# mll-lab-nu/TStar

Hardware: AMD Instinct MI355X
Metric: candidate frames scored/sec (whole node) + sec/video to 8 keyframes, 1h@1fps (higher is better)
Workload: dtype f32 held exactly as 3 bf16 terms per operand: every GEMM and vision-attention operand (activations, weights, Q, K, V, softmax probabilities) = three round-to-nearest bf16 terms carrying all 24 significand bits; the 6 partial products with i + j <= 2 (each exact) on v_mfma_f32_32x32x16_bf16, f32 accu

## Files before the change

### tstar_amd/csrc/attention_x3.h

```cpp
#pragma once
#include <hip/hip_runtime.h>
#include <math.h>
#include <utility>

namespace tstar {
namespace ax3 {

typedef __bf16 bf16x8 __attribute__((ext_vector_type(8)));
typedef __bf16 bf16x2 __attribute__((ext_vector_type(2)));
typedef float f32x2 __attribute__((ext_vector_type(2)));
typedef float f32x4 __attribute__((ext_vector_type(4)));
typedef float f32x16 __attribute__((ext_vector_type(16)));
typedef unsigned int u32x4 __attribute__((ext_vector_type(4)));
typedef unsigned int u32x2 __attribute__((ext_vector_type(2)));

constexpr int HD = 64, KB = 32;
constexpr int VPITCH = 80;
constexpr int KP = KB * 128, VP = HD * VPITCH;
constexpr int KBUF = 3 * KP, VBUF = 3 * VP, NKB = 2, NVB = 3;
constexpr int LDS_BYTES = NKB * KBUF + NVB * VBUF;

#define AX3_FENCE() __builtin_amdgcn_sched_barrier(0)

__device__ __forceinline__ void split2_rn3(float x0, float x1, unsigned (&o)[3]) {
#pragma unroll
    for (int k = 0; k < 3; ++k) {
        f32x2 x; x[0] = x0; x[1] = x1;
        const unsigned hb = __builtin_bit_cast(unsigned, __builtin_convertvector(x, bf16x2));
        o[k] = hb;
        if (k < 2) {
            x0 = x0 - __uint_as_float(hb << 16);
            x1 = x1 - __uint_as_float(hb & 0xFFFF0000u);
        }
    }
}
__device__ __forceinline__ float xhalf_max(float x) {
    const auto r = __builtin_amdgcn_permlane32_swap(__float_as_uint(x), __float_as_uint(x), false, false);
    return fmaxf(__uint_as_float(r[0]), __uint_as_float(r[1]));
}
__device__ __forceinline__ float xhalf_sum(float x) {
    const auto r = __builtin_amdgcn_permlane32_swap(__float_as_uint(x), __float_as_uint(x), false, false);
    return __uint_as_float(r[0]) + __uint_as_float(r[1]);
}

__device__ __forceinline__ int k_off(int key, int chunk) { return key * 128 + ((chunk ^ ((key >> 1) & 7)) << 4); }
__device__ __forceinline__ int v_off(int d, int chunk) { return d * VPITCH + (chunk << 4); }
__device__ __forceinline__ int v_keypos(int k) { const int g = k >> 2; const int gp = (g & 4) | ((g & 1) << 1) | ((g >> 1) & 1); return (gp * 4 + (k & 3)) * 2; }

__device__ __forceinline__ f32x16 mfma(const bf16x8 a, const u32x4 b, const f32x16 c) {
    return __builtin_amdgcn_mfma_f32_32x32x16_bf16(a, __builtin_bit_cast(bf16x8, b), c, 0, 0, 0);
}

template <bool PLANES>
__global__ __launch_bounds__(256, 2) void attention_x3_kernel(const float* __restrict__ qkv, const char* __restrict__ planes,
                                                              float* __restrict__ out, int T, int heads, int qtiles) {
    extern __shared__ __attribute__((aligned(16))) char smem[];
    char* const kbuf = smem;
    char* const vbuf = smem + NKB * KBUF;

    const int D = heads * HD, D3 = 3 * D;
    int bid = blockIdx.x;
    const int qt = bid % qtiles; bid /= qtiles;
    const int head = bid % heads;
    const int b = bid / heads;

    const int t = threadIdx.x, lane = t & 63, wave = __builtin_amdgcn_readfirstlane(t >> 6);
    const int l31 = lane & 31, h = lane >> 5;
    const size_t rowbase = (size_t)b * T;

    const int q = qt * 128 + wave * 32 + l31;
    const int qc = q < T ? q : T - 1;
    const bool wave_active = (qt * 128 + wave * 32) < T;

    u32x4 qp[3][4];
    {
        const float* src = qkv + (rowbase + qc) * D3 + head * HD + 8 * h;
        const float sc = 0.125f * 1.44269504088896340736f;
#pragma unroll
        for (int s = 0; s < 4; ++s) {
            const f32x4 a = *reinterpret_cast<const f32x4*>(src + 16 * s) * sc;
            const f32x4 c = *reinterpret_cast<const f32x4*>(src + 16 * s + 4) * sc;
            unsigned o0[3], o1[3], o2[3], o3[3];
            split2_rn3(a[0], a[1], o0); split2_rn3(a[2], a[3], o1); split2_rn3(c[0], c[1], o2); split2_rn3(c[2], c[3], o3);
#pragma unroll
            for (int k = 0; k < 3; ++k) { qp[k][s][0] = o0[k]; qp[k][s][1] = o1[k]; qp[k][s][2] = o2[k]; qp[k][s][3] = o3[k]; }
        }
    }

    const int kc4 = t & 15, kr = t >> 4;
    const int vkp = t & 15, vdq = t >> 4;
    const __amdgpu_buffer_rsrc_t kv_rsrc =
        __builtin_amdgcn_make_buffer_rsrc(const_cast<float*>(qkv + rowbase * D3), 0, (int)((size_t)T * D3 * 4), 0x00020000);
    int kvo[2], vvo[2];
#pragma unroll
    for (int i = 0; i < 2; ++i) {
        kvo[i] = ((kr + 16 * i) * D3 + D + head * HD + kc4 * 4) * 4;
        vvo[i] = ((2 * vkp + i) * D3 + 2 * D + head * HD + vdq * 4) * 4;
    }
    const int kwr0 = k_off(kr, kc4 >> 1) + (kc4 & 1) * 8, kwr1 = k_off(kr + 16, kc4 >> 1) + (kc4 & 1) * 8;
    int vwr[4];
#pragma unroll
    for (int e = 0; e < 4; ++e) {
        const int pos = v_keypos(2 * vkp);
        vwr[e] = v_off(4 * vdq + e, pos >> 4) + (pos & 15);
    }

    const int R0 = b * T;
    const int kt0 = R0 >> 5;
    const bool tail_key = !PLANES && (T % KB) == 1;
    const int nkb = PLANES ? ((R0 + T - 1) >> 5) - kt0 + 1 : (tail_key ? T / KB : (T + KB - 1) / KB);

    f32x4 rk[2], rv[2];
    auto gload = [&](int kb) __attribute__((always_inline)) {
        const int so = (kb < nkb ? kb : nkb) * (KB * 4) * D3;
#pragma unroll
        for (int i = 0; i < 2; ++i) {
            rk[i] = __builtin_bit_cast(f32x4, __builtin_amdgcn_raw_buffer_load_b128(kv_rsrc, kvo[i], so, 0));
            rv[i] = __builtin_bit_cast(f32x4, __builtin_amdgcn_raw_buffer_load_b128(kv_rsrc, vvo[i], so, 0));
        }
    };
    unsigned ksp[2][3];
    auto stage_piece = [&](auto P, char* kdst, char* vdst) __attribute__((always_inline)) {
        constexpr int p = decltype(P)::value;
        if constexpr (p < 4) {
            constexpr int i = p >> 1, hf = p & 1;
            split2_rn3(rk[i][2 * hf], rk[i][2 * hf + 1], ksp[hf]);
            if constexpr (hf == 1) {
#pragma unroll
                for (int k = 0; k < 3; ++k) {
                    u32x2 v; v[0] = ksp[0][k]; v[1] = ksp[1][k];
                    *reinterpret_cast<u32x2*>(kdst + k * KP + (i == 0 ? kwr0 : kwr1)) = v;
                }
            }
        } else {
            constexpr int e = p - 4;
            unsigned o[3];
            split2_rn3(rv[0][e], rv[1][e], o);
#pragma unroll
            for (int k = 0; k < 3; ++k) *reinterpret_cast<unsigned*>(vdst + k * VP + vwr[e]) = o[k];
        }
    };
    auto stage_all = [&](int kb) __attribute__((always_inline)) {
        char* kd = kbuf + (kb & 1) * KBUF;
        char* vd = vbuf + (kb % NVB) * VBUF;
        [&]<int... P>(std::integer_sequence<int, P...>) __attribute__((always_inline)) {
            (stage_piece(std::integral_constant<int, P>{}, kd, vd), ...);
        }(std::make_integer_sequence<int, 8>{});
    };

    auto dma = [&](int kb) __attribute__((always_inline)) {
        if constexpr (PLANES) {
            if (kb < nkb) {
                const char* src = planes + ((size_t)(kt0 + kb) * heads + head) * (size_t)(KBUF + VBUF) + lane * 16;
                const unsigned kdst = (unsigned)(size_t)(kbuf + (kb & 1) * KBUF), vdst = (unsigned)(size_t)(vbuf + (kb % NVB) * VBUF);
                constexpr int NCH = (KBUF + VBUF) / 1024;
                static_assert((KBUF + VBUF) % 1024 == 0 && KBUF % 1024 == 0, "tile images are copied in 1-KB wave loads");
#pragma unroll
                for (int c = 0; c < (NCH + 3) / 4; ++c) {
                    const int chunk = wave + 4 * c;
                    if (chunk >= NCH) break;
                    const unsigned dst = __builtin_amdgcn_readfirstlane(chunk < KBUF / 1024 ? kdst + chunk * 1024 : vdst + (chunk - KBUF / 1024) * 1024);
                    const char* g = src + chunk * 1024;
                    unsigned keep;
                    asm volatile("s_mov_b32 %0, m0\n\ts_mov_b32 m0, %2\n\ts_nop 0\n\tglobal_load_lds_dwordx4 %1, off\n\ts_mov_b32 m0, %0"
                                 : "=&s"(keep) : "v"(g), "s"(dst) : "memory");
                }
            }
        }
    };

    int kro[4], vro[2];
#pragma unroll
    for (int s = 0; s < 4; ++s) kro[s] = k_off(l31, 2 * s + h);
#pragma unroll
    for (int ks = 0; ks < 2; ++ks) vro[ks] = v_off(l31, 2 * ks + h);
    auto rdk = [&](const char* kb_, int plane, int s) __attribute__((always_inline)) {
        return *reinterpret_cast<const bf16x8*>(kb_ + plane * KP + kro[s]);
    };
    auto rdv = [&](const char* vb_, int plane, int dt, int ks) __attribute__((always_inline)) {
        return *reinterpret_cast<const bf16x8*>(vb_ + plane * VP + dt * (32 * VPITCH) + vro[ks]);
    };

    f32x16 zero16;
#pragma unroll
    for (int r = 0; r < 16; ++r) zero16[r] = 0.f;
    f32x16 o0, o1, s0_, s1_;
#pragma unroll
    for (int r = 0; r < 16; ++r) { o0[r] = 0.f; o1[r] = 0.f; s0_[r] = 0.f; s1_[r] = 0.f; }
    float m_run = -INFINITY, l_run = 0.f, alpha = 1.f, m_new = 0.f, ps = 0.f, mb = 0.f;
    u32x4 pp[3][2];
    bf16x8 vf[3][2];

    if constexpr (PLANES) {
        dma(0);
        dma(1);
        asm volatile("s_waitcnt vmcnt(0)" ::: "memory");
    } else if (nkb > 0) {
        gload(0);
        stage_all(0);
        gload(1);
        if (nkb > 1) stage_all(1);
        gload(2);
    }
    __syncthreads();
    if (wave_active && nkb > 0) {
#pragma unroll
        for (int s = 0; s < 4; ++s) {
            const bf16x8 k0 = rdk(kbuf, 0, s), k1 = rdk(kbuf, 1, s), k2 = rdk(kbuf, 2, s);
            s0_ = mfma(k0, qp[2][s], s0_); s0_ = mfma(k0, qp[1][s], s0_);
            s0_ = mfma(k0, qp[0][s], s0_); s0_ = mfma(k1, qp[1][s], s0_);
            s0_ = mfma(k1, qp[0][s], s0_); s0_ = mfma(k2, qp[0][s], s0_);
        }
    }
    __syncthreads();

    auto soft_piece = [&](auto P, auto MASK, f32x16& sc_, int kb) __attribute__((always_inline)) {
        constexpr int p = decltype(P)::value;
        if constexpr (p == 0) {
            if constexpr (PLANES) {
                if (decltype(MASK)::value) {
                    const int row0 = (kt0 + kb) * KB + 4 * h - R0;
#pragma unroll
                    for (int r = 0; r < 16; ++r) sc_[r] = (unsigned)(row0 + (r & 3) + 8 * (r >> 2)) < (unsigned)T ? sc_[r] : -INFINITY;
                }
            } else if (decltype(MASK)::value && !tail_key && kb == nkb - 1) {
                const int key0 = kb * KB + 4 * h;
#pragma unroll
                for (int r = 0; r < 16; ++r) sc_[r] = (key0 + (r & 3) + 8 * (r >> 2)) < T ? sc_[r] : -INFINITY;
            }
            mb = sc_[0];
#pragma unroll
            for (int r = 1; r < 16; ++r) mb = fmaxf(mb, sc_[r]);
        } else if constexpr (p == 1) {
            mb = xhalf_max(mb);
            m_new = fmaxf(m_run, mb);
            alpha = __builtin_amdgcn_exp2f(m_run - m_new);
            m_run = m_new;
            ps = 0.f;
        } else if constexpr (p < 6) {
            constexpr int c = p - 2;
#pragma unroll
            for (int r = 4 * c; r < 4 * c + 4; ++r) { sc_[r] = __builtin_amdgcn_exp2f(sc_[r] - m_new); ps += sc_[r]; }
        } else if constexpr (p == 6) {
            ps = xhalf_sum(ps);
            l_run = l_run * alpha + ps;
        } else {
            constexpr int j = p - 7;
            unsigned o[3];
            split2_rn3(sc_[2 * j], sc_[2 * j + 1], o);
#pragma unroll
            for (int k = 0; k < 3; ++k) pp[k][j >> 2][j & 3] = o[k];
        }
    };

    auto phase_a = [&](auto DOQK, auto MASK, f32x16& sc_, f32x16& sn, int kb) __attribute__((always_inline)) {
        constexpr bool doqk = decltype(DOQK)::value;
        const char* kb_ = kbuf + ((kb + 1) & 1) * KBUF;
        bf16x8 k0, k1, k2;
        if constexpr (doqk) {
            k0 = rdk(kb_, 0, 0); k1 = rdk(kb_, 1, 0); k2 = rdk(kb_, 2, 0);
        }
        soft_piece(std::integral_constant<int, 0>{}, MASK, sc_, kb);
        AX3_FENCE();
        [&]<int... S>(std::integer_sequence<int, S...>) __attribute__((always_inline)) {
            ([&] {
                if constexpr (doqk) { sn = mfma(k0, qp[2][S], S == 0 ? zero16 : sn); sn = mfma(k0, qp[1][S], sn); }
                soft_piece(std::integral_constant<int, 1 + 3 * S>{}, MASK, sc_, kb);
                AX3_FENCE();
                if constexpr (doqk) {
                    sn = mfma(k0, qp[0][S], sn);
                    if constexpr (S < 3) k0 = rdk(kb_, 0, S + 1);
                    sn = mfma(k1, qp[1][S], sn);
                }
                soft_piece(std::integral_constant<int, 2 + 3 * S>{}, MASK, sc_, kb);
                AX3_FENCE();
                if constexpr (doqk) {
                    sn = mfma(k1, qp[0][S], sn);
                    if constexpr (S < 3) k1 = rdk(kb_, 1, S + 1);
                    sn = mfma(k2, qp[0][S], sn);
                    if constexpr (S < 3) k2 = rdk(kb_, 2, S + 1);
                }
                soft_piece(std::integral_constant<int, 3 + 3 * S>{}, MASK, sc_, kb);
                AX3_FENCE();
            }(), ...);
        }(std::make_integer_sequence<int, 4>{});
        {
            const char* vb_ = vbuf + (kb % NVB) * VBUF;
#pragma unroll
            for (int k = 0; k < 3; ++k) { vf[k][0] = rdv(vb_, k, 0, 0); vf[k][1] = rdv(vb_, k, 1, 0); }
        }
        soft_piece(std::integral_constant<int, 13>{}, MASK, sc_, kb);
        soft_piece(std::integral_constant<int, 14>{}, MASK, sc_, kb);
        AX3_FENCE();
    };

    auto phase_b = [&](auto DOST, int kb) __attribute__((always_inline)) {
        constexpr bool dost = decltype(DOST)::value;
        const char* vb_ = vbuf + (kb % NVB) * VBUF;
        char* kd = kbuf + (kb & 1) * KBUF;
        char* vd = vbuf + ((kb + 2) % NVB) * VBUF;
        if (!__all(alpha == 1.0f)) {
#pragma unroll
            for (int r = 0; r < 16; ++r) { o0[r] *= alpha; o1[r] *= alpha; }
        }
        AX3_FENCE();
        auto extra = [&](auto G) __attribute__((always_inline)) {
            constexpr int g = decltype(G)::value;
            if constexpr (dost && !PLANES) {
                if constexpr (g < 8) stage_piece(std::integral_constant<int, g>{}, kd, vd);
                if constexpr (g == 8) gload(kb + 3);
            }
            AX3_FENCE();
        };
        [&]<int... KS>(std::integer_sequence<int, KS...>) __attribute__((always_inline)) {
            ([&] {
                o0 = mfma(vf[0][0], pp[2][KS], o0); o1 = mfma(vf[0][1], pp[2][KS], o1);
                extra(std::integral_constant<int, 6 * KS + 0>{});
                o0 = mfma(vf[0][0], pp[1][KS], o0); o1 = mfma(vf[0][1], pp[1][KS], o1);
                extra(std::integral_constant<int, 6 * KS + 1>{});
                o0 = mfma(vf[0][0], pp[0][KS], o0); o1 = mfma(vf[0][1], pp[0][KS], o1);
                if constexpr (KS == 0) { vf[0][0] = rdv(vb_, 0, 0, 1); vf[0][1] = rdv(vb_, 0, 1, 1); }
                extra(std::integral_constant<int, 6 * KS + 2>{});
                o0 = mfma(vf[1][0], pp[1][KS], o0); o1 = mfma(vf[1][1], pp[1][KS], o1);
                extra(std::integral_constant<int, 6 * KS + 3>{});
                o0 = mfma(vf[1][0], pp[0][KS], o0); o1 = mfma(vf[1][1], pp[0][KS], o1);
                if constexpr (KS == 0) { vf[1][0] = rdv(vb_, 1, 0, 1); vf[1][1] = rdv(vb_, 1, 1, 1); }
                extra(std::integral_constant<int, 6 * KS + 4>{});
                o0 = mfma(vf[2][0], pp[0][KS], o0); o1 = mfma(vf[2][1], pp[0][KS], o1);
                if constexpr (KS == 0) { vf[2][0] = rdv(vb_, 2, 0, 1); vf[2][1] = rdv(vb_, 2, 1, 1); }
                extra(std::integral_constant<int, 6 * KS + 5>{});
            }(), ...);
        }(std::make_integer_sequence<int, 2>{});
    };

    auto tile_barrier = [&]() __attribute__((always_inline)) {
        if constexpr (PLANES) asm volatile("s_waitcnt vmcnt(0) lgkmcnt(0)" ::: "memory");
        else asm volatile("s_waitcnt lgkmcnt(0)" ::: "memory");
        __builtin_amdgcn_s_barrier();
        AX3_FENCE();
    };
    auto iteration = [&](int kb) __attribute__((always_inline)) {
        dma(kb + 2);
        if (kb & 1) { if (kb + 1 < nkb) phase_a(std::true_type{}, std::true_type{}, s1_, s0_, kb); else phase_a(std::false_type{}, std::true_type{}, s1_, s0_, kb); }
        else { if (kb + 1 < nkb) phase_a(std::true_type{}, std::true_type{}, s0_, s1_, kb); else phase_a(std::false_type{}, std::true_type{}, s0_, s1_, kb); }
        if (kb + 2 < nkb) phase_b(std::true_type{}, kb); else phase_b(std::false_type{}, kb);
        tile_barrier();
    };
    if (wave_active) {
        __builtin_amdgcn_s_setprio(1);
        int kb = 0;
        if constexpr (PLANES) {
            if (nkb > 0) { iteration(0); kb = 1; }
            for (; kb + 2 < nkb; kb += 2) {
                dma(kb + 2);
                phase_a(std::true_type{}, std::false_type{}, s1_, s0_, kb);
                phase_b(std::true_type{}, kb);
                tile_barrier();
                dma(kb + 3);
                phase_a(std::true_type{}, std::false_type{}, s0_, s1_, kb + 1);
                phase_b(std::true_type{}, kb + 1);
                tile_barrier();
            }
        } else {
            for (; kb + 3 < nkb; kb += 2) {
                phase_a(std::true_type{}, std::false_type{}, s0_, s1_, kb);
                phase_b(std::true_type{}, kb);
                tile_barrier();
                phase_a(std::true_type{}, std::false_type{}, s1_, s0_, kb + 1);
                phase_b(std::true_type{}, kb + 1);
                tile_barrier();
            }
        }
        for (; kb < nkb; ++kb) iteration(kb);
        __builtin_amdgcn_s_setprio(0);
    } else {
        for (int kb = 0; kb < nkb; ++kb) {
            if constexpr (PLANES) dma(kb + 2);
            else if (kb + 2 < nkb) { stage_all(kb + 2); gload(kb + 3); }
            tile_barrier();
        }
    }

    if (tail_key && wave_active) {
        const size_t ro = (rowbase + (T - 1)) * D3 + head * HD;
        float sx = 0.f;
#pragma unroll
        for (int s = 0; s < 4; ++s) {
            const f32x4 k0 = *reinterpret_cast<const f32x4*>(qkv + ro + D + 16 * s + 8 * h);
            const f32x4 k1 = *reinterpret_cast<const f32x4*>(qkv + ro + D + 16 * s + 8 * h + 4);
#pragma unroll
            for (int e = 0; e < 8; ++e) {
                auto term = [&](int k) { const unsigned dw = qp[k][s][e >> 1]; return __uint_as_float((e & 1) ? (dw & 0xFFFF0000u) : (dw << 16)); };
                const float qv = (term(0) + term(1)) + term(2);
                sx += (e < 4 ? k0[e] : k1[e - 4]) * qv;
            }
        }
        sx = xhalf_sum(sx);
        const float mn = fmaxf(m_run, sx);
        const float al = __builtin_amdgcn_exp2f(m_run - mn);
        const float p = __builtin_amdgcn_exp2f(sx - mn);
        l_run = l_run * al + p;
        m_run = mn;
#pragma unroll
        for (int g4 = 0; g4 < 4; ++g4) {
            const f32x4 v0 = *reinterpret_cast<const f32x4*>(qkv + ro + 2 * D + 8 * g4 + 4 * h);
            const f32x4 v1 = *reinterpret_cast<const f32x4*>(qkv + ro + 2 * D + 32 + 8 * g4 + 4 * h);
#pragma unroll
            for (int e = 0; e < 4; ++e) {
                o0[g4 * 4 + e] = o0[g4 * 4 + e] * al + p * v0[e];
                o1[g4 * 4 + e] = o1[g4 * 4 + e] * al + p * v1[e];
            }
        }
    }

    if (q < T) {
        const float inv = 1.0f / l_run;
        float* op = out + (rowbase + q) * D + head * HD + 4 * h;
#pragma unroll
        for (int g4 = 0; g4 < 4; ++g4) {
            f32x4 a, c;
#pragma unroll
            for (int e = 0; e < 4; ++e) { a[e] = o0[g4 * 4 + e] * inv; c[e] = o1[g4 * 4 + e] * inv; }
            *reinterpret_cast<f32x4*>(op + 8 * g4) = a;
            *reinterpret_cast<f32x4*>(op + 32 + 8 * g4) = c;
        }
    }
}

}

inline size_t kv_planes_bytes(int rows, int heads) { return (size_t)((rows + 31) / 32) * heads * (size_t)(ax3::KBUF + ax3::VBUF); }

#ifdef TSTAR_ATTN_X3_LAB
namespace ax3 {
__global__ __launch_bounds__(256) void kv_planes_kernel(const float* __restrict__ qkv, char* __restrict__ planes, int rows, int heads) {
    const int D = heads * HD, D3 = 3 * D;
    const size_t gid = (size_t)blockIdx.x * 256 + threadIdx.x;
    const int dq = (int)(gid % 16), head = (int)((gid / 16) % heads);
    const size_t rp = gid / (16 * (size_t)heads);
    const int row = (int)(rp * 2);
    if (row >= ((rows + 31) / 32) * 32) return;
    const int kt = row >> 5, key = row & 31;
    char* tile = planes + ((size_t)kt * heads + head) * (size_t)(KBUF + VBUF);
    f32x4 kx[2], vx[2];
#pragma unroll
    for (int i = 0; i < 2; ++i) {
        if (row + i < rows) {
            kx[i] = *reinterpret_cast<const f32x4*>(qkv + (size_t)(row + i) * D3 + D + head * HD + dq * 4);
            vx[i] = *reinterpret_cast<const f32x4*>(qkv + (size_t)(row + i) * D3 + 2 * D + head * HD + dq * 4);
        } else {
            kx[i] = f32x4{0.f, 0.f, 0.f, 0.f};
            vx[i] = f32x4{0.f, 0.f, 0.f, 0.f};
        }
    }
#pragma unroll
    for (int i = 0; i < 2; ++i) {
        unsigned o0[3], o1[3];
        split2_rn3(kx[i][0], kx[i][1], o0);
        split2_rn3(kx[i][2], kx[i][3], o1);
#pragma unroll
        for (int k = 0; k < 3; ++k) {
            u32x2 v; v[0] = o0[k]; v[1] = o1[k];
            *reinterpret_cast<u32x2*>(tile + k * KP + k_off(key + i, dq >> 1) + (dq & 1) * 8) = v;
        }
    }
    const int pos = v_keypos(key);
#pragma unroll
    for (int e = 0; e < 4; ++e) {
        unsigned o[3];
        split2_rn3(vx[0][e], vx[1][e], o);
#pragma unroll
        for (int k = 0; k < 3; ++k) *reinterpret_cast<unsigned*>(tile + KBUF + k * VP + v_off(4 * dq + e, pos >> 4) + (pos & 15)) = o[k];
    }
}
}
#endif

inline int attention_x3_launch(const float* qkv, float* out, int B, int T, int heads, hipStream_t s, const char* planes = nullptr) {
    const int qtiles = (T + 127) / 128;
#ifdef TSTAR_ATTN_X3_LAB
    static bool attr[2] = {false, false};
    if (planes) {
        if (!attr[1]) {
            const hipError_t e = hipFuncSetAttribute(reinterpret_cast<const void*>(ax3::attention_x3_kernel<true>), hipFuncAttributeMaxDynamicSharedMemorySize, ax3::LDS_BYTES);
            if (e != hipSuccess) return (int)e;
            attr[1] = true;
        }
        hipLaunchKernelGGL(ax3::attention_x3_kernel<true>, dim3(B * heads * qtiles), dim3(256), ax3::LDS_BYTES, s, qkv, planes, out, T, heads, qtiles);
        return (int)hipGetLastError();
    }
    if (!attr[0]) {
        const hipError_t e = hipFuncSetAttribute(reinterpret_cast<const void*>(ax3::attention_x3_kernel<false>), hipFuncAttributeMaxDynamicSharedMemorySize, ax3::LDS_BYTES);
        if (e != hipSuccess) return (int)e;
        attr[0] = true;
    }
#endif
    if (planes) return (int)hipErrorInvalidValue;
    hipLaunchKernelGGL(ax3::attention_x3_kernel<false>, dim3(B * heads * qtiles), dim3(256), ax3::LDS_BYTES, s, qkv, planes, out, T, heads, qtiles);
    return (int)hipGetLastError();
}

#ifdef TSTAR_ATTN_X3_LAB
inline int kv_planes_launch(const float* qkv, char* planes, int rows, int heads, hipStream_t s) {
    const size_t n = (size_t)((rows + 31) / 32) * 16 * 16 * heads;
    hipLaunchKernelGGL(ax3::kv_planes_kernel, dim3((unsigned)((n + 255) / 256)), dim3(256), 0, s, qkv, planes, rows, heads);
    return (int)hipGetLastError();
}
#endif

}
```

Baseline: 11890.

## Finely interleave softmax exp and bf16 split steps between attention MFMAs

Replaces the coarse softmax pieces with a per-MFMA gap schedule. Each exponential and each sub-step of the 3-term bf16 split now sits in its own slot between QK MFMAs, with inline-asm register pins to hold the order. The splits of the last probability pairs (set by SPLIT_A) move into phase B alongside the PV MFMAs, and the V-fragment LDS reads are redistributed so latency is hidden behind MFMAs. The aim is to remove VALU/MFMA serialization stalls in the attention inner loop, at the cost of more live registers and reliance on the compiler honoring the pinned schedule. Optional timestamp instrumentation is added behind lab macros.

```diff
diff --git a/tstar_amd/csrc/attention_x3.h b/tstar_amd/csrc/attention_x3.h
--- a/tstar_amd/csrc/attention_x3.h
+++ b/tstar_amd/csrc/attention_x3.h
@@ -21,6 +21,24 @@
 constexpr int LDS_BYTES = NKB * KBUF + NVB * VBUF;
 
 #define AX3_FENCE() __builtin_amdgcn_sched_barrier(0)
+template <class V> __device__ __forceinline__ void pin(V& x) { asm volatile("" : "+v"(x)); }
+
+#ifndef AX3_SPLIT_A
+#define AX3_SPLIT_A 6
+#endif
+constexpr int SPLIT_STEPS = 11, SPLIT_A = AX3_SPLIT_A;
+constexpr int STAGE_G0 = 8 - SPLIT_A < 2 ? 8 - SPLIT_A : 2;
+constexpr int split_begin(int g) {
+    const int b = g < 2 ? 0 : g <= 17 ? 2 * (g - 2) : g <= 23 ? 32 + 6 * (g - 18) : SPLIT_A * SPLIT_STEPS;
+    return b < SPLIT_A * SPLIT_STEPS ? b : SPLIT_A * SPLIT_STEPS;
+}
+constexpr bool split_follows_exps() {
+    for (int j = 0; j < SPLIT_A; ++j)
+        if (split_begin(2 * j + 2) > j * SPLIT_STEPS) return false;
+    return true;
+}
+static_assert(SPLIT_A >= 4 && SPLIT_A <= 8, "the pairs 0..3 feed the first MFMA of phase B; the others only its K = 16 step 1 (group 6 on)");
+static_assert(split_follows_exps(), "a pair is split before its exponentials");
 
 __device__ __forceinline__ void split2_rn3(float x0, float x1, unsigned (&o)[3]) {
 #pragma unroll
@@ -50,6 +68,13 @@
 __device__ __forceinline__ f32x16 mfma(const bf16x8 a, const u32x4 b, const f32x16 c) {
     return __builtin_amdgcn_mfma_f32_32x32x16_bf16(a, __builtin_bit_cast(bf16x8, b), c, 0, 0, 0);
 }
+
+#if defined(TSTAR_ATTN_X3_LAB) && defined(AX3_STAMPS)
+__device__ unsigned long long ax3_stamps[4];
+#define AX3_STAMP(i) do { const unsigned long long now_ = __builtin_amdgcn_s_memtime(); stamp_acc[i] += now_ - stamp_last; stamp_last = now_; } while (0)
+#else
+#define AX3_STAMP(i) do { } while (0)
+#endif
 
 template <bool PLANES>
 __global__ __launch_bounds__(256, 2) void attention_x3_kernel(const float* __restrict__ qkv, const char* __restrict__ planes,
@@ -214,84 +239,112 @@
     }
     __syncthreads();
 
-    auto soft_piece = [&](auto P, auto MASK, f32x16& sc_, int kb) __attribute__((always_inline)) {
-        constexpr int p = decltype(P)::value;
-        if constexpr (p == 0) {
-            if constexpr (PLANES) {
-                if (decltype(MASK)::value) {
-                    const int row0 = (kt0 + kb) * KB + 4 * h - R0;
-#pragma unroll
-                    for (int r = 0; r < 16; ++r) sc_[r] = (unsigned)(row0 + (r & 3) + 8 * (r >> 2)) < (unsigned)T ? sc_[r] : -INFINITY;
-                }
-            } else if (decltype(MASK)::value && !tail_key && kb == nkb - 1) {
-                const int key0 = kb * KB + 4 * h;
-#pragma unroll
-                for (int r = 0; r < 16; ++r) sc_[r] = (key0 + (r & 3) + 8 * (r >> 2)) < T ? sc_[r] : -INFINITY;
-            }
-            mb = sc_[0];
-#pragma unroll
-            for (int r = 1; r < 16; ++r) mb = fmaxf(mb, sc_[r]);
-        } else if constexpr (p == 1) {
-            mb = xhalf_max(mb);
-            m_new = fmaxf(m_run, mb);
-            alpha = __builtin_amdgcn_exp2f(m_run - m_new);
-            m_run = m_new;
-            ps = 0.f;
-        } else if constexpr (p < 6) {
-            constexpr int c = p - 2;
-#pragma unroll
-            for (int r = 4 * c; r < 4 * c + 4; ++r) { sc_[r] = __builtin_amdgcn_exp2f(sc_[r] - m_new); ps += sc_[r]; }
-        } else if constexpr (p == 6) {
-            ps = xhalf_sum(ps);
-            l_run = l_run * alpha + ps;
-        } else {
-            constexpr int j = p - 7;
-            unsigned o[3];
-            split2_rn3(sc_[2 * j], sc_[2 * j + 1], o);
-#pragma unroll
-            for (int k = 0; k < 3; ++k) pp[k][j >> 2][j & 3] = o[k];
-        }
+    auto p_max = [&](auto MASK, f32x16& sc_, int kb) __attribute__((always_inline)) {
+        if constexpr (PLANES) {
+            if (decltype(MASK)::value) {
+                const int row0 = (kt0 + kb) * KB + 4 * h - R0;
+#pragma unroll
+                for (int r = 0; r < 16; ++r) sc_[r] = (unsigned)(row0 + (r & 3) + 8 * (r >> 2)) < (unsigned)T ? sc_[r] : -INFINITY;
+            }
+        } else if (decltype(MASK)::value && !tail_key && kb == nkb - 1) {
+            const int key0 = kb * KB + 4 * h;
+#pragma unroll
+            for (int r = 0; r < 16; ++r) sc_[r] = (key0 + (r & 3) + 8 * (r >> 2)) < T ? sc_[r] : -INFINITY;
+        }
+        mb = sc_[0];
+#pragma unroll
+        for (int r = 1; r < 16; ++r) mb = fmaxf(mb, sc_[r]);
+        pin(mb);
+    };
+    auto p_stat = [&]() __attribute__((always_inline)) {
+        mb = xhalf_max(mb);
+        m_new = fmaxf(m_run, mb);
+        alpha = __builtin_amdgcn_exp2f(m_run - m_new);
+        m_run = m_new;
+        ps = 0.f;
+        pin(m_new); pin(alpha);
+    };
+    auto p_sum = [&]() __attribute__((always_inline)) {
+        ps = xhalf_sum(ps);
+        l_run = l_run * alpha + ps;
+        pin(l_run);
+    };
+    float sx0[8], sx1[8], st_[8];
+    unsigned shb[8][3];
+    auto split_step = [&](auto J, auto S, f32x16& sc_) __attribute__((always_inline)) {
+        constexpr int j = decltype(J)::value, s = decltype(S)::value, k = s / 5, w = s % 5;
+        constexpr bool first = k == 0 && j < SPLIT_A;
+        const float x0 = first ? sc_[2 * j] : sx0[j], x1 = first ? sc_[2 * j + 1] : sx1[j];
+        if constexpr (w == 0) {
+            f32x2 x; x[0] = x0; x[1] = x1;
+            shb[j][k] = __builtin_bit_cast(unsigned, __builtin_convertvector(x, bf16x2));
+        } else if constexpr (w == 1) st_[j] = __uint_as_float(shb[j][k] << 16);
+        else if constexpr (w == 2) sx0[j] = x0 - st_[j];
+        else if constexpr (w == 3) st_[j] = __uint_as_float(shb[j][k] & 0xFFFF0000u);
+        else sx1[j] = x1 - st_[j];
+    };
+    auto split_pin = [&](auto J, auto S) __attribute__((always_inline)) {
+        constexpr int j = decltype(J)::value, s = decltype(S)::value, k = s / 5, w = s % 5;
+        if constexpr (w == 0) { pin(shb[j][k]); pp[k][j >> 2][j & 3] = shb[j][k]; }
+        else if constexpr (w == 1 || w == 3) pin(st_[j]);
+        else if constexpr (w == 2) pin(sx0[j]);
+        else pin(sx1[j]);
+    };
+    auto split_steps = [&]<int... P>(std::integer_sequence<int, P...>, auto BASE, f32x16& sc_) __attribute__((always_inline)) {
+        (split_step(std::integral_constant<int, (decltype(BASE)::value + P) / SPLIT_STEPS>{},
+                    std::integral_constant<int, (decltype(BASE)::value + P) % SPLIT_STEPS>{}, sc_), ...);
+        (split_pin(std::integral_constant<int, (decltype(BASE)::value + P) / SPLIT_STEPS>{},
+                   std::integral_constant<int, (decltype(BASE)::value + P) % SPLIT_STEPS>{}), ...);
+    };
+    auto gap_a = [&](auto G, f32x16& sc_) __attribute__((always_inline)) {
+        constexpr int g = decltype(G)::value;
+        AX3_FENCE();
+        if constexpr (g == 0) p_stat();
+        if constexpr (g >= 1 && g <= 16) sc_[g - 1] = __builtin_amdgcn_exp2f(sc_[g - 1] - m_new);
+        if constexpr (g == 17) p_sum();
+        split_steps(std::make_integer_sequence<int, split_begin(g + 1) - split_begin(g)>{}, std::integral_constant<int, split_begin(g)>{}, sc_);
+        if constexpr (g >= 1 && g <= 16) { pin(sc_); ps += sc_[g - 1]; pin(ps); }
+        AX3_FENCE();
     };
 
     auto phase_a = [&](auto DOQK, auto MASK, f32x16& sc_, f32x16& sn, int kb) __attribute__((always_inline)) {
         constexpr bool doqk = decltype(DOQK)::value;
         const char* kb_ = kbuf + ((kb + 1) & 1) * KBUF;
+        const char* vb_ = vbuf + (kb % NVB) * VBUF;
         bf16x8 k0, k1, k2;
         if constexpr (doqk) {
             k0 = rdk(kb_, 0, 0); k1 = rdk(kb_, 1, 0); k2 = rdk(kb_, 2, 0);
         }
-        soft_piece(std::integral_constant<int, 0>{}, MASK, sc_, kb);
+        p_max(MASK, sc_, kb);
         AX3_FENCE();
         [&]<int... S>(std::integer_sequence<int, S...>) __attribute__((always_inline)) {
             ([&] {
-                if constexpr (doqk) { sn = mfma(k0, qp[2][S], S == 0 ? zero16 : sn); sn = mfma(k0, qp[1][S], sn); }
-                soft_piece(std::integral_constant<int, 1 + 3 * S>{}, MASK, sc_, kb);
-                AX3_FENCE();
+                if constexpr (doqk) sn = mfma(k0, qp[2][S], S == 0 ? zero16 : sn);
+                gap_a(std::integral_constant<int, 6 * S + 0>{}, sc_);
+                if constexpr (doqk) sn = mfma(k0, qp[1][S], sn);
+                gap_a(std::integral_constant<int, 6 * S + 1>{}, sc_);
                 if constexpr (doqk) {
                     sn = mfma(k0, qp[0][S], sn);
                     if constexpr (S < 3) k0 = rdk(kb_, 0, S + 1);
-                    sn = mfma(k1, qp[1][S], sn);
                 }
-                soft_piece(std::integral_constant<int, 2 + 3 * S>{}, MASK, sc_, kb);
-                AX3_FENCE();
+                gap_a(std::integral_constant<int, 6 * S + 2>{}, sc_);
+                if constexpr (doqk) sn = mfma(k1, qp[1][S], sn);
+                gap_a(std::integral_constant<int, 6 * S + 3>{}, sc_);
                 if constexpr (doqk) {
                     sn = mfma(k1, qp[0][S], sn);
                     if constexpr (S < 3) k1 = rdk(kb_, 1, S + 1);
+                }
+                gap_a(std::integral_constant<int, 6 * S + 4>{}, sc_);
+                if constexpr (doqk) {
                     sn = mfma(k2, qp[0][S], sn);
                     if constexpr (S < 3) k2 = rdk(kb_, 2, S + 1);
                 }
-                soft_piece(std::integral_constant<int, 3 + 3 * S>{}, MASK, sc_, kb);
-                AX3_FENCE();
+                if constexpr (S == 3) { vf[0][0] = rdv(vb_, 0, 0, 0); vf[0][1] = rdv(vb_, 0, 1, 0); }
+                gap_a(std::integral_constant<int, 6 * S + 5>{}, sc_);
             }(), ...);
         }(std::make_integer_sequence<int, 4>{});
-        {
-            const char* vb_ = vbuf + (kb % NVB) * VBUF;
-#pragma unroll
-            for (int k = 0; k < 3; ++k) { vf[k][0] = rdv(vb_, k, 0, 0); vf[k][1] = rdv(vb_, k, 1, 0); }
-        }
-        soft_piece(std::integral_constant<int, 13>{}, MASK, sc_, kb);
-        soft_piece(std::integral_constant<int, 14>{}, MASK, sc_, kb);
-        AX3_FENCE();
+#pragma unroll
+        for (int j = SPLIT_A; j < 8; ++j) { sx0[j] = sc_[2 * j]; sx1[j] = sc_[2 * j + 1]; }
     };
 
     auto phase_b = [&](auto DOST, int kb) __attribute__((always_inline)) {
@@ -306,15 +359,21 @@
         AX3_FENCE();
         auto extra = [&](auto G) __attribute__((always_inline)) {
             constexpr int g = decltype(G)::value;
+            if constexpr (g < 8 - SPLIT_A)
+                split_steps(std::make_integer_sequence<int, SPLIT_STEPS>{}, std::integral_constant<int, (SPLIT_A + g) * SPLIT_STEPS>{}, s0_);
             if constexpr (dost && !PLANES) {
-                if constexpr (g < 8) stage_piece(std::integral_constant<int, g>{}, kd, vd);
-                if constexpr (g == 8) gload(kb + 3);
+                if constexpr (g >= STAGE_G0 && g < STAGE_G0 + 8) stage_piece(std::integral_constant<int, g - STAGE_G0>{}, kd, vd);
+                if constexpr (g == STAGE_G0 + 8) gload(kb + 3);
             }
             AX3_FENCE();
         };
         [&]<int... KS>(std::integer_sequence<int, KS...>) __attribute__((always_inline)) {
             ([&] {
                 o0 = mfma(vf[0][0], pp[2][KS], o0); o1 = mfma(vf[0][1], pp[2][KS], o1);
+                if constexpr (KS == 0) {
+#pragma unroll
+                    for (int k = 1; k < 3; ++k) { vf[k][0] = rdv(vb_, k, 0, 0); vf[k][1] = rdv(vb_, k, 1, 0); }
+                }
                 extra(std::integral_constant<int, 6 * KS + 0>{});
                 o0 = mfma(vf[0][0], pp[1][KS], o0); o1 = mfma(vf[0][1], pp[1][KS], o1);
                 extra(std::integral_constant<int, 6 * KS + 1>{});
@@ -339,12 +398,18 @@
         __builtin_amdgcn_s_barrier();
         AX3_FENCE();
     };
+#if defined(TSTAR_ATTN_X3_LAB) && defined(AX3_STAMPS)
+    unsigned long long stamp_acc[3] = {0, 0, 0}, stamp_last = __builtin_amdgcn_s_memtime();
+#endif
     auto iteration = [&](int kb) __attribute__((always_inline)) {
         dma(kb + 2);
         if (kb & 1) { if (kb + 1 < nkb) phase_a(std::true_type{}, std::true_type{}, s1_, s0_, kb); else phase_a(std::false_type{}, std::true_type{}, s1_, s0_, kb); }
         else { if (kb + 1 < nkb) phase_a(std::true_type{}, std::true_type{}, s0_, s1_, kb); else phase_a(std::false_type{}, std::true_type{}, s0_, s1_, kb); }
+        AX3_STAMP(0);
         if (kb + 2 < nkb) phase_b(std::true_type{}, kb); else phase_b(std::false_type{}, kb);
+        AX3_STAMP(1);
         tile_barrier();
+        AX3_STAMP(2);
     };
     if (wave_active) {
         __builtin_amdgcn_s_setprio(1);
@@ -353,26 +418,33 @@
             if (nkb > 0) { iteration(0); kb = 1; }
             for (; kb + 2 < nkb; kb += 2) {
                 dma(kb + 2);
-                phase_a(std::true_type{}, std::false_type{}, s1_, s0_, kb);
-                phase_b(std::true_type{}, kb);
-                tile_barrier();
+                phase_a(std::true_type{}, std::false_type{}, s1_, s0_, kb); AX3_STAMP(0);
+                phase_b(std::true_type{}, kb); AX3_STAMP(1);
+                tile_barrier(); AX3_STAMP(2);
                 dma(kb + 3);
-                phase_a(std::true_type{}, std::false_type{}, s0_, s1_, kb + 1);
-                phase_b(std::true_type{}, kb + 1);
-                tile_barrier();
+                phase_a(std::true_type{}, std::false_type{}, s0_, s1_, kb + 1); AX3_STAMP(0);
+                phase_b(std::true_type{}, kb + 1); AX3_STAMP(1);
+                tile_barrier(); AX3_STAMP(2);
             }
         } else {
             for (; kb + 3 < nkb; kb += 2) {
-                phase_a(std::true_type{}, std::false_type{}, s0_, s1_, kb);
-                phase_b(std::true_type{}, kb);
-                tile_barrier();
-                phase_a(std::true_type{}, std::false_type{}, s1_, s0_, kb + 1);
-                phase_b(std::true_type{}, kb + 1);
-                tile_barrier();
+                phase_a(std::true_type{}, std::false_type{}, s0_, s1_, kb); AX3_STAMP(0);
+                phase_b(std::true_type{}, kb); AX3_STAMP(1);
+                tile_barrier(); AX3_STAMP(2);
+                phase_a(std::true_type{}, std::false_type{}, s1_, s0_, kb + 1); AX3_STAMP(0);
+                phase_b(std::true_type{}, kb + 1); AX3_STAMP(1);
+                tile_barrier(); AX3_STAMP(2);
             }
         }
         for (; kb < nkb; ++kb) iteration(kb);
         __builtin_amdgcn_s_setprio(0);
+#if defined(TSTAR_ATTN_X3_LAB) && defined(AX3_STAMPS)
+        if (lane == 0) {
+#pragma unroll
+            for (int i = 0; i < 3; ++i) atomicAdd(&ax3_stamps[i], stamp_acc[i]);
+            atomicAdd(&ax3_stamps[3], (unsigned long long)nkb);
+        }
+#endif
     } else {
         for (int kb = 0; kb < nkb; ++kb) {
             if constexpr (PLANES) dma(kb + 2);
```

New measurement: 11940 (median of 6 runs). No clear change (+0.5%).
